# jiwoon-ahn/irn

Measured on AMD Instinct MI355X. Metric: images/sec for CAM+random-walk label gen, VOC12 512^2 (random-walk label generation stage), higher is better.
Workload: dtype f32

## Files before the change

include/irn_hip.h:

```cpp
#ifndef IRN_HIP_H
#define IRN_HIP_H

#include <stddef.h>
#include <stdint.h>

#ifdef __cplusplus
extern "C" {
#endif

#define IRN_OK 0
#define IRN_ERR_ARG 1
#define IRN_ERR_HIP 2
#define IRN_ERR_STATE 3

#define IRN_MAX_RADIUS 16

int irn_version(void);
const char *irn_last_error(void);

int irn_path_count(int radius, int *n_dirs, int *n_cells);
int irn_path_table(int radius, int order, int32_t *dst_dydx, int32_t *path_start, int32_t *cells_dydx);

int irn_edge_to_affinity(const float *edge_dev, int batch, int hp, int wp, int radius,
                         float *aff_dev, void *stream);
// ... 23 lines not shown
                       const int32_t *c, size_t *workspace_bytes);
int irn_walk_run(irn_walk_ctx *ctx, const float *const *edge_dev, const float *const *cam_dev,
                 const int32_t *const *inst_map_dev, const int32_t *k_inst,
                 float *const *out_dev, float beta, int n_sweeps,
                 void *workspace_dev, size_t workspace_bytes, void *stream);

int irn_walk_steps(irn_walk_ctx *ctx, int n_sweeps, int *n_steps);
int irn_power_series(int n, int tol_exp, double *coef_out, int coef_cap, int *n_steps, int *recurrence);

int irn_walk_set_option(irn_walk_ctx *ctx, const char *name, int value);

int irn_walk_sync(irn_walk_ctx *ctx, int *fell_back);
int irn_walk_check(irn_walk_ctx *ctx);
int irn_walk_fallback_runs(irn_walk_ctx *ctx);

int irn_walk_tuning(irn_walk_ctx *ctx, int *poll_delay, int *placement, float *probe_ms4);

int irn_walk_plan_rounds(int radius, int n_images, const int32_t *h, const int32_t *w, const int32_t *channels,
                         int n_workgroups, int placement, int32_t *jobs_out, int cap_rounds, int *n_rounds);

int irn_walk_read_profile(irn_walk_ctx *ctx, long long *host_out);

int irn_walk_enable_timing(irn_walk_ctx *ctx, int enable);
int irn_walk_last_sweep_ms(irn_walk_ctx *ctx, float *ms, int *n_launches);

int irn_walk_export_weights(irn_walk_ctx *ctx, int image, float *w_dev, double *inv_deg_dev,
                            void *workspace_dev, void *stream);

int irn_label_epilogue(int n_images, const float *const *rw_dev, const int32_t *c, const int32_t *h,
                       const int32_t *w, const int32_t *out_h, const int32_t *out_w, float bg_thres,
                       const int64_t *const *keys_dev, uint8_t *const *labels_dev,
                       int32_t *const *argmax_dev, float *const *rw_up_dev, void *scratch_dev,
                       void *stream);

int irn_cam_merge(int n_scales, const float *const *src_dev, const int32_t *hs, const int32_t *ws, int n_classes,
                  const int64_t *keys_dev, int n_keys, int out_h, int out_w, float *cam_dev, float *high_res_dev,
                  void *scratch_dev, void *stream);

int irn_bicubic_plan(int in_size, int out_size, int32_t *ksize, int32_t *lo, int32_t *count, int32_t *weights,
                     size_t weights_capacity);
size_t irn_bicubic_scratch_bytes(int h, int w, int hs, int ws, int channels);
int irn_bicubic_resize_u8(const uint8_t *img_dev, int h, int w, int channels, int hs, int ws, uint8_t *out_dev,
                          void *scratch_dev, void *stream);
int irn_msf_pack(const uint8_t *img_dev, int h, int w, int n_scales, const int32_t *hs, const int32_t *ws,
                 const float *lut_dev, float *const *out_dev, void *scratch_dev, void *stream);

#define IRN_AUGMENT_DESC_WORDS 16
int irn_augment_batch(int n_images, int crop, const int32_t *meta, size_t meta_words, const uint8_t *pixels_dev,
                      size_t pixels_bytes, const float *lut_dev, float *out_dev, size_t out_elems, void *scratch_dev,
                      size_t scratch_bytes, int32_t *meta_dev, size_t meta_dev_words, void *stream);

#define IRN_AUGMENT_LABEL_DESC_WORDS 12
int irn_augment_label_batch(int n_images, int crop, int reduce, const int32_t *meta, size_t meta_words,
                            const uint8_t *labels_dev, size_t labels_bytes, uint8_t *out_dev, size_t out_elems,
                            int32_t *meta_dev, size_t meta_dev_words, void *stream);

int irn_bn_act(float *x_dev, const float *res_dev, const float *scale_dev, const float *shift_dev, const float *res_scale_dev,
               const float *res_shift_dev, int64_t n_images, int n_channels, int64_t plane_elems, int relu, void *stream);

int irn_bn_act_nhwc(float *x_dev, const float *res_dev, const float *scale_dev, const float *shift_dev, const float *res_scale_dev,
                    const float *res_shift_dev, int64_t n_pixels, int n_channels, int relu, void *stream);

int irn_bn_fold(const float *weight_dev, const float *bias_dev, const float *mean_dev, const float *var_dev, double eps,
                int n_channels, float *scale_dev, float *shift_dev, void *stream);
int irn_bn_act_forward(const float *x_dev, const float *res_dev, const float *scale_dev, const float *shift_dev,
                       const float *res_scale_dev, const float *res_shift_dev, float *out_dev, int64_t n_images, int n_channels,
// ... 118 lines not shown
```

irn_amd/_lib.py:

```python
import ctypes as C
import os

import torch

_HERE = os.path.dirname(os.path.abspath(__file__))
LIB_PATH = os.environ.get("IRN_HIP_LIB") or os.path.join(_HERE, "lib", "libirn_hip.so")

if not os.path.exists(LIB_PATH):
    raise ImportError(
        "irn_amd: %s not found — the HIP extension is the product path and has no fallback; "
        "build it with `make -C irn_amd/csrc` (needs hipcc, targets gfx950)" % LIB_PATH)

lib = C.CDLL(LIB_PATH)

vp, i32, f32, sz, i64 = C.c_void_p, C.c_int, C.c_float, C.c_size_t, C.c_int64
pi32 = C.POINTER(C.c_int32)
ppv = C.POINTER(C.c_void_p)

_SIGS = {
    "irn_version": (C.c_int, []),
    "irn_last_error": (C.c_char_p, []),
    "irn_path_count": (i32, [i32, C.POINTER(i32), C.POINTER(i32)]),
    "irn_path_table": (i32, [i32, i32, pi32, pi32, pi32]),
    "irn_edge_to_affinity": (i32, [vp, i32, i32, i32, i32, vp, vp]),
    "irn_edge_to_affinity_backward": (i32, [vp, vp, i32, i32, i32, i32, vp, vp]),
    "irn_pair_displacement": (i32, [vp, i32, i32, i32, i32, i32, vp, vp]),
    "irn_pair_displacement_backward": (i32, [vp, i32, i32, i32, i32, i32, vp, vp]),
    "irn_aff_loss_workspace_bytes": (sz, [i32, i32, i32, i32]),
    "irn_aff_loss_forward": (i32, [vp, vp, vp, i32, i32, i32, i32, vp, vp, vp, sz, vp]),
    "irn_aff_loss_backward": (i32, [vp, vp, vp, i32, i32, i32, i32, vp, vp, vp, vp, sz, vp]),
    "irn_aff_loss_backward_ordered": (i32, [vp, vp, vp, i32, i32, i32, i32, vp, vp, vp, vp, sz, vp]),
    "irn_walk_create": (i32, [i32, C.POINTER(vp)]),
    "irn_walk_destroy": (i32, [vp]),
    "irn_walk_configure": (i32, [vp, i32, pi32, pi32, pi32, C.POINTER(sz)]),
    "irn_walk_run": (i32, [vp, ppv, ppv, ppv, pi32, ppv, f32, i32, vp, sz, vp]),
    "irn_walk_set_option": (i32, [vp, C.c_char_p, i32]),
    "irn_walk_steps": (i32, [vp, i32, C.POINTER(i32)]),
    "irn_power_series": (i32, [i32, i32, C.POINTER(C.c_double), i32, C.POINTER(i32), C.POINTER(i32)]),
    "irn_walk_sync": (i32, [vp, C.POINTER(i32)]),
    "irn_walk_check": (i32, [vp]),
    "irn_walk_fallback_runs": (i32, [vp]),
    "irn_walk_tuning": (i32, [vp, C.POINTER(i32), C.POINTER(i32), C.POINTER(f32)]),
    "irn_walk_plan_rounds": (i32, [i32, i32, pi32, pi32, pi32, i32, i32, pi32, i32, C.POINTER(i32)]),
    "irn_walk_read_profile": (i32, [vp, vp]),
    "irn_walk_enable_timing": (i32, [vp, i32]),
    "irn_walk_last_sweep_ms": (i32, [vp, C.POINTER(f32), C.POINTER(i32)]),
    "irn_walk_export_weights": (i32, [vp, i32, vp, vp, vp, vp]),
    "irn_label_epilogue": (i32, [i32, ppv, pi32, pi32, pi32, pi32, pi32, f32, ppv, ppv, ppv, ppv, vp, vp]),
    "irn_cam_merge": (i32, [i32, ppv, pi32, pi32, i32, vp, i32, i32, i32, vp, vp, vp, vp]),
    "irn_bicubic_plan": (i32, [i32, i32, pi32, pi32, pi32, pi32, sz]),
    "irn_bicubic_scratch_bytes": (sz, [i32, i32, i32, i32, i32]),
    "irn_bicubic_resize_u8": (i32, [vp, i32, i32, i32, i32, i32, vp, vp, vp]),
    "irn_msf_pack": (i32, [vp, i32, i32, i32, pi32, pi32, vp, ppv, vp, vp]),
    "irn_augment_batch": (i32, [i32, i32, pi32, sz, vp, sz, vp, vp, sz, vp, sz, vp, sz, vp]),
    "irn_augment_label_batch": (i32, [i32, i32, i32, pi32, sz, vp, sz, vp, sz, vp, sz, vp]),
    "irn_bn_act": (i32, [vp, vp, vp, vp, vp, vp, i64, i32, i64, i32, vp]),
    "irn_bn_act_nhwc": (i32, [vp, vp, vp, vp, vp, vp, i64, i32, i32, vp]),
    "irn_bn_fold": (i32, [vp, vp, vp, vp, C.c_double, i32, vp, vp, vp]),
    "irn_bn_act_forward": (i32, [vp, vp, vp, vp, vp, vp, vp, i64, i32, i64, i32, vp]),
    "irn_bn_act_backward_workspace_bytes": (sz, [i64, i32, i64]),
    "irn_bn_act_backward": (i32, [vp, vp, vp, vp, vp, vp, vp, vp, vp, i64, i32, i64, i32, vp, sz, vp]),
    "irn_conv1x1_workspace_bytes": (sz, []),
    "irn_conv1x1_algo_count": (i32, [i64, i32, i32, i32, i32, i32, sz, C.POINTER(i32)]),
    "irn_conv1x1_nhwc": (i32, [vp, vp, vp, vp, vp, i64, i32, i32, i32, i32, vp, sz, vp]),
    "irn_split16": (i32, [vp, vp, vp, i32, vp, i64, i32, vp, vp]),
    "irn_split16_pad": (i32, [vp, vp, vp, i32, vp, i64, i32, i32, i32, i32, i32, vp, vp]),
    "irn_conv3x3_split_gemm": (i32, [vp, vp, vp, i64, i32, i32, i32, i32, f32, i32, i32, vp, sz, vp]),
    "irn_gemm16_algo_count": (i32, [i64, i32, i32, i32, i32, i32, sz, C.POINTER(i32)]),
    "irn_gemm16_nhwc": (i32, [vp, vp, vp, vp, vp, i64, i32, i32, i32, f32, i32, vp, sz, vp]),
    "irn_stem_pool": (i32, [vp, vp, vp, i64, i32, i32, i32, vp, vp]),
    "irn_upsample_bilinear": (i32, [vp, i64, i32, i32, i32, i32, vp, vp]),
    "irn_upsample_bilinear_backward": (i32, [vp, vp, i64, i32, i32, i32, i32, vp, vp]),
    "irn_find_centroids": (i32, [vp, i32, i32, i32, vp, vp]),
    "irn_cluster_scratch_bytes": (sz, [i32, i32]),
    "irn_cluster_centroids": (i32, [vp, vp, i32, i32, f32, vp, C.POINTER(i32), vp, vp]),
    "irn_find_centroids_batch": (i32, [i32, ppv, pi32, pi32, i32, ppv, vp]),
    "irn_cluster_batch_scratch_bytes": (sz, [i32, pi32, pi32]),
    "irn_cluster_centroids_batch": (i32, [i32, ppv, ppv, pi32, pi32, f32, ppv, vp, vp, vp]),
    "irn_ccl_scratch_bytes": (sz, [i32, i32, i32]),
    "irn_label4": (i32, [vp, i32, i32, i32, vp, vp, vp, vp]),
    "irn_detect_scratch_bytes": (sz, [i32, i32, i32]),
# ... 70 lines not shown
```

irn_amd/csrc/label.hip:

```cpp
#include "kernels.hpp"

#pragma clang fp contract(off)

namespace irn {

struct LabelJob {
    const float *rw;
    const int64_t *keys;
    uint8_t *labels;
    int32_t *argmax;
    float *rw_up;
    unsigned *max_slot;
    int c, h, w, oh, ow;
    const uint8_t *gt;
};

namespace {

__device__ __forceinline__ unsigned enc_ordered(float f) {
    const unsigned b = __float_as_uint(f);
    return (b & 0x80000000u) ? ~b : (b | 0x80000000u);
}
__device__ __forceinline__ float dec_ordered(unsigned u) {
    return __uint_as_float((u & 0x80000000u) ? (u & 0x7fffffffu) : ~u);
}

struct Taps {
    int i0, i1;
    float l0, l1;
};

__device__ __forceinline__ Taps taps_x4(int dst, int n_in) {
    float src = ((float)dst + 0.5f) * 0.25f;
    src = src - 0.5f;
    src = src < 0.f ? 0.f : src;
    Taps t;
    t.i0 = min((int)src, n_in - 1);
    t.i1 = min(t.i0 + 1, n_in - 1);
    t.l1 = src - (float)t.i0;
    t.l0 = 1.0f - t.l1;
    return t;
}

__device__ __forceinline__ float bilerp(const float *__restrict__ plane, int w, const Taps &ty, const Taps &tx) {
    const float v00 = plane[ty.i0 * w + tx.i0], v01 = plane[ty.i0 * w + tx.i1];
    const float v10 = plane[ty.i1 * w + tx.i0], v11 = plane[ty.i1 * w + tx.i1];
    const float p01 = v01 * tx.l1, p11 = v11 * tx.l1;
    const float top = __builtin_fmaf(v00, tx.l0, p01);
    const float bot = __builtin_fmaf(v10, tx.l0, p11);
    const float pb = ty.l1 * bot;
    return __builtin_fmaf(ty.l0, top, pb);
}

__device__ __forceinline__ int cell_lo(int k) { return k == 0 ? 0 : 4 * k + 2; }

template <int PASS>
__global__ __launch_bounds__(256) void upsample_max_kernel(const LabelJob *__restrict__ jobs) {
    const LabelJob J = jobs[blockIdx.y];
    const unsigned plane_px = (unsigned)(J.h * J.w), cells = (unsigned)J.c * plane_px;
    const float lower = PASS == 2 ? dec_ordered(*J.max_slot) : 0.f;
    float m = -INFINITY;
    for (unsigned i = blockIdx.x * 256 + threadIdx.x; i < cells; i += gridDim.x * 256) {
        const int c = (int)(i / plane_px);
        const int r = (int)(i - (unsigned)c * plane_px);
        const int k = (int)((unsigned)r / (unsigned)J.w), l = r - k * J.w;
        const int y0 = cell_lo(k), x0 = cell_lo(l);
        if (y0 >= J.oh || x0 >= J.ow) continue;
        const float *plane = J.rw + (long)c * J.h * J.w;
        if (PASS == 1) {
            m = fmaxf(m, bilerp(plane, J.w, taps_x4(y0, J.h), taps_x4(x0, J.w)));
        } else {
            const int k1 = min(k + 1, J.h - 1), l1 = min(l + 1, J.w - 1);
            const float u = fmaxf(fmaxf(plane[k * J.w + l], plane[k * J.w + l1]), fmaxf(plane[k1 * J.w + l], plane[k1 * J.w + l1]));
            if (u + fabsf(u) * 1e-6f + 1e-37f < lower) continue;
            const int y1 = min(k == J.h - 1 ? 4 * J.h - 1 : 4 * k + 5, J.oh - 1);
            const int x1 = min(l == J.w - 1 ? 4 * J.w - 1 : 4 * l + 5, J.ow - 1);
            for (int oy = y0; oy <= y1; ++oy) {
                const Taps ty = taps_x4(oy, J.h);
                for (int ox = x0; ox <= x1; ++ox) m = fmaxf(m, bilerp(plane, J.w, ty, taps_x4(ox, J.w)));
            }
        }
    }
    for (int s = 32; s > 0; s >>= 1) m = fmaxf(m, __shfl_xor(m, s));
    __shared__ float wmax[4];
    if ((threadIdx.x & 63) == 0) wmax[threadIdx.x >> 6] = m;
    __syncthreads();
    if (threadIdx.x == 0) {
        m = fmaxf(fmaxf(wmax[0], wmax[1]), fmaxf(wmax[2], wmax[3]));
        if (m > -INFINITY) atomicMax(J.max_slot, enc_ordered(m));
    }
}

__device__ __forceinline__ float bilerp_vals(float v00, float v01, float v10, float v11, const Taps &ty, const Taps &tx) {
    const float p01 = v01 * tx.l1, p11 = v11 * tx.l1;
    const float top = __builtin_fmaf(v00, tx.l0, p01);
    const float bot = __builtin_fmaf(v10, tx.l0, p11);
    const float pb = ty.l1 * bot;
    return __builtin_fmaf(ty.l0, top, pb);
}

__global__ __launch_bounds__(256) void label_argmax_kernel(const LabelJob *__restrict__ jobs, float bg) {
    const LabelJob J = jobs[blockIdx.y];
    const unsigned gw = (unsigned)(J.ow + 3) >> 2, groups = gw * (unsigned)J.oh;
    const unsigned npx = (unsigned)J.oh * (unsigned)J.ow;
    const float gmax = dec_ordered(*J.max_slot);
    for (unsigned g = blockIdx.x * 256 + threadIdx.x; g < groups; g += gridDim.x * 256) {
        const int oy = (int)(g / gw), ox = (int)(g - (unsigned)oy * gw) * 4;
        const int nq = min(4, J.ow - ox);
        const Taps ty = taps_x4(oy, J.h);
        Taps tx[4];
#pragma unroll
        for (int q = 0; q < 4; ++q) tx[q] = taps_x4(min(ox + q, J.ow - 1), J.w);
        float best[4] = {bg, bg, bg, bg};
        int idx[4] = {0, 0, 0, 0};
        const unsigned o = (unsigned)oy * (unsigned)J.ow + (unsigned)ox;
        for (int c = 0; c < J.c; ++c) {
            const float *r0 = J.rw + (long)c * J.h * J.w + ty.i0 * J.w, *r1 = J.rw + (long)c * J.h * J.w + ty.i1 * J.w;
            const float a00 = r0[tx[0].i0], a01 = r0[tx[0].i1], a10 = r1[tx[0].i0], a11 = r1[tx[0].i1];
// ... 5 lines not shown
            v[3] = bilerp_vals(b00, b01, b10, b11, ty, tx[3]) / gmax;
            if (J.rw_up) {
                float *dst = J.rw_up + (long)c * npx + o;
                if (nq == 4 && ((uintptr_t)dst & 15) == 0) *reinterpret_cast<float4 *>(dst) = make_float4(v[0], v[1], v[2], v[3]);
                else
                    for (int q = 0; q < nq; ++q) dst[q] = v[q];
            }
#pragma unroll
            for (int q = 0; q < 4; ++q)
                if (v[q] > best[q] || (v[q] != v[q] && best[q] == best[q])) {
                    best[q] = v[q];
                    idx[q] = c + 1;
                }
        }
        if (J.argmax) {
            int32_t *dst = J.argmax + o;
            if (nq == 4 && ((uintptr_t)dst & 15) == 0) *reinterpret_cast<int4 *>(dst) = make_int4(idx[0], idx[1], idx[2], idx[3]);
            else
                for (int q = 0; q < nq; ++q) dst[q] = idx[q];
        }
        if (J.labels) {
            uint8_t lab[4];
#pragma unroll
            for (int q = 0; q < 4; ++q) lab[q] = idx[q] == 0 ? (uint8_t)0 : (uint8_t)(J.keys[idx[q] - 1] + 1);
            uint8_t *dst = J.labels + o;
            if (nq == 4 && ((uintptr_t)dst & 3) == 0)
                *reinterpret_cast<uint32_t *>(dst) = (uint32_t)lab[0] | ((uint32_t)lab[1] << 8) | ((uint32_t)lab[2] << 16) | ((uint32_t)lab[3] << 24);
            else
                for (int q = 0; q < nq; ++q) dst[q] = lab[q];
        }
    }
}

constexpr int kSweepGroups = 4;
constexpr int kSweepChunk = 256 * kSweepGroups;
constexpr int kSweepCap = 15360;
constexpr int kSweepRows = IRN_EVAL_CLASSES + 1;
constexpr int kSweepMaxC = IRN_EVAL_CLASSES - 1;
constexpr uint32_t kSweepSkip = 0xffffffffu;

__global__ __launch_bounds__(256) void label_sweep_kernel(const LabelJob *__restrict__ jobs, const float *__restrict__ thres,
                                                          int t, int cap, int64_t *__restrict__ hist, int64_t *__restrict__ bad) {
    extern __shared__ __attribute__((aligned(16))) uint32_t sweep_lds[];
    uint32_t *bins = sweep_lds;
    float *th = reinterpret_cast<float *>(sweep_lds + cap);
    int *col = reinterpret_cast<int *>(th + IRN_EVAL_MAX_THRES);
    uint32_t *nbad = reinterpret_cast<uint32_t *>(col + kSweepMaxC);
    const LabelJob J = jobs[blockIdx.y];
    const int tid = threadIdx.x;
    if (tid == 0) *nbad = 0;
    for (int i = tid; i < t; i += 256) th[i] = thres[i];
    if (tid < J.c) {
        const int64_t key = J.keys[tid];
        col[tid] = (key >= 0 && key < kSweepMaxC) ? (int)key + 1 : -1;
    }
    __syncthreads();
    uint32_t local_bad = 0;
    if (blockIdx.x == 0 && blockIdx.y == 0)
        for (int i = tid; i < t; i += 256)
            if (th[i] != th[i] || (i > 0 && !(th[i - 1] <= th[i]))) ++local_bad;

    const unsigned gw = (unsigned)(J.ow + 3) >> 2, groups = gw * (unsigned)J.oh;
    const unsigned chunks = (groups + kSweepChunk - 1) / kSweepChunk;
    const uint32_t nbins = (uint32_t)(t + 1) * kSweepRows * (uint32_t)J.c;
    const float gmax = dec_ordered(*J.max_slot);
    for (unsigned chunk = blockIdx.x; chunk < chunks; chunk += gridDim.x) {
// ... 122 lines not shown
        const int oy = (int)(o / ow), ox = (int)(o - (long)oy * ow);
        float acc = 0.f;
        for (int s = 0; s < A.n_scales; ++s) {
            const Taps ty = taps_resize(oy, A.hs[s], th), tx = taps_resize(ox, A.ws[s], tw);
            acc = acc + bilerp(A.src[s] + (long)cls * A.hs[s] * A.ws[s], A.ws[s], ty, tx);
        }
        out[o] = acc;
        m = fmaxf(m, acc);
    }
    for (int s = 32; s > 0; s >>= 1) m = fmaxf(m, __shfl_xor(m, s));
    __shared__ float wmax[4];
    if ((threadIdx.x & 63) == 0) wmax[threadIdx.x >> 6] = m;
    __syncthreads();
    if (threadIdx.x == 0) {
        m = fmaxf(fmaxf(wmax[0], wmax[1]), fmaxf(wmax[2], wmax[3]));
        if (m > -INFINITY) atomicMax(A.max_slots + (is_hi ? A.k : 0) + kk, enc_ordered(m));
    }
}

__global__ __launch_bounds__(256) void cam_merge_norm_kernel(const MergeArgs A) {
    const int kk = blockIdx.y;
    const bool is_hi = blockIdx.z == 1;
    const long n = is_hi ? (long)A.H * A.W : (long)A.lh * A.lw;
    float *out = (is_hi ? A.hi : A.lo) + (long)kk * n;
    const float den = dec_ordered(A.max_slots[(is_hi ? A.k : 0) + kk]) + 1e-5f;
    for (long o = (long)blockIdx.x * 256 + threadIdx.x; o < n; o += (long)gridDim.x * 256) out[o] = out[o] / den;
}

}
}

using namespace irn;

extern "C" int irn_label_epilogue(int n_images, const float *const *rw_dev, const int32_t *c, const int32_t *h,
                                  const int32_t *w, const int32_t *out_h, const int32_t *out_w, float bg_thres,
                                  const int64_t *const *keys_dev, uint8_t *const *labels_dev,
                                  int32_t *const *argmax_dev, float *const *rw_up_dev, void *scratch_dev,
                                  void *stream_) {
    hipStream_t stream = (hipStream_t)stream_;
    if (n_images < 1 || !rw_dev || !c || !h || !w || !out_h || !out_w || !scratch_dev)
        return fail(IRN_ERR_ARG, "irn_label_epilogue: bad argument");
    std::vector<LabelJob> jobs(n_images);
    long max_px = 0, max_cells = 0;
    for (int i = 0; i < n_images; ++i) {
        LabelJob &J = jobs[i];
        if (!rw_dev[i] || c[i] < 1 || h[i] < 1 || w[i] < 1 || out_h[i] < 1 || out_w[i] < 1 ||
            out_h[i] > 4 * h[i] || out_w[i] > 4 * w[i])
            return fail(IRN_ERR_ARG, "irn_label_epilogue: image %d: bad sizes (c=%d %dx%d -> %dx%d)", i, c[i], h[i],
                        w[i], out_h[i], out_w[i]);
        J.rw = rw_dev[i];
        J.keys = keys_dev ? keys_dev[i] : nullptr;
        J.labels = labels_dev ? labels_dev[i] : nullptr;
        J.argmax = argmax_dev ? argmax_dev[i] : nullptr;
        J.rw_up = rw_up_dev ? rw_up_dev[i] : nullptr;
        if (J.labels && !J.keys)
            return fail(IRN_ERR_ARG, "irn_label_epilogue: image %d: labels requested without keys", i);
        J.max_slot = (unsigned *)scratch_dev + i;
        J.c = c[i]; J.h = h[i]; J.w = w[i]; J.oh = out_h[i]; J.ow = out_w[i];
        max_px = std::max(max_px, (long)out_h[i] * out_w[i]);
        max_cells = std::max(max_cells, (long)c[i] * h[i] * w[i]);
    }
    LabelJob *jobs_dev = nullptr;
    int rc = scratch_upload(jobs.data(), sizeof(LabelJob) * n_images, (void **)&jobs_dev, stream);
    if (rc) return rc;
    IRN_HIP_TRY(hipMemsetAsync(scratch_dev, 0, sizeof(unsigned) * n_images, stream));
    if (max_px >= (1L << 31) || max_cells >= (1L << 31)) return fail(IRN_ERR_ARG, "irn_label_epilogue: image too large (32-bit pixel indices)");
    const long per_image = std::max<long>(1, 4096 / n_images);
    const int bx = (int)std::min<long>((max_px / 4 + 255) / 256 + 1, 512);
    const int bc = (int)std::min<long>((max_cells + 255) / 256, per_image);
    hipLaunchKernelGGL(upsample_max_kernel<1>, dim3(bc, n_images), dim3(256), 0, stream, jobs_dev);
    IRN_LAUNCH_CHECK("upsample_max_kernel<1>");
    hipLaunchKernelGGL(upsample_max_kernel<2>, dim3(bc, n_images), dim3(256), 0, stream, jobs_dev);
    IRN_LAUNCH_CHECK("upsample_max_kernel<2>");
    hipLaunchKernelGGL(label_argmax_kernel, dim3(bx, n_images), dim3(256), 0, stream, jobs_dev, bg_thres);
    IRN_LAUNCH_CHECK("label_argmax_kernel");
    return scratch_release(stream);
}

extern "C" int irn_label_sweep_confusion(int n_images, const float *const *rw_dev, const int32_t *c, const int32_t *h,
                                         const int32_t *w, const int32_t *out_h, const int32_t *out_w,
                                         const int64_t *const *keys_dev, const uint8_t *const *gt_dev,
                                         const float *thres_dev, int t, int64_t *hist_dev, int64_t *bad_dev,
                                         void *scratch_dev, void *stream_) {
    hipStream_t stream = (hipStream_t)stream_;
    if (n_images < 1 || n_images > 65535 || !rw_dev || !c || !h || !w || !out_h || !out_w || !keys_dev || !gt_dev || !thres_dev ||
        !hist_dev || !bad_dev || !scratch_dev || t < 1 || t > IRN_EVAL_MAX_THRES)
        return fail(IRN_ERR_ARG, "irn_label_sweep_confusion: bad argument (n_images=%d, t=%d; 1 <= t <= %d)", n_images, t,
                    IRN_EVAL_MAX_THRES);
    std::vector<LabelJob> jobs(n_images);
    long max_px = 0, max_cells = 0;
    int max_c = 0;
    for (int i = 0; i < n_images; ++i) {
        LabelJob &J = jobs[i];
        if (!rw_dev[i] || c[i] < 1 || c[i] > kSweepMaxC || h[i] < 1 || w[i] < 1 || out_h[i] < 1 || out_w[i] < 1 ||
            out_h[i] > 4 * h[i] || out_w[i] > 4 * w[i])
            return fail(IRN_ERR_ARG, "irn_label_sweep_confusion: image %d: bad sizes (c=%d %dx%d -> %dx%d; 1 <= c <= %d)", i,
                        c[i], h[i], w[i], out_h[i], out_w[i], kSweepMaxC);
        if (!keys_dev[i] || !gt_dev[i])
            return fail(IRN_ERR_ARG, "irn_label_sweep_confusion: image %d: keys and ground truth are required", i);
        J.rw = rw_dev[i];
        J.keys = keys_dev[i];
        J.labels = nullptr;
        J.argmax = nullptr;
        J.rw_up = nullptr;
        J.gt = gt_dev[i];
        J.max_slot = (unsigned *)scratch_dev + i;
        J.c = c[i]; J.h = h[i]; J.w = w[i]; J.oh = out_h[i]; J.ow = out_w[i];
        max_px = std::max(max_px, (long)out_h[i] * out_w[i]);
        max_cells = std::max(max_cells, (long)c[i] * h[i] * w[i]);
        max_c = std::max(max_c, c[i]);
    }
    if (max_px >= (1L << 31) || max_cells >= (1L << 31))
        return fail(IRN_ERR_ARG, "irn_label_sweep_confusion: image too large (32-bit pixel indices)");
    LabelJob *jobs_dev = nullptr;
    int rc = scratch_upload(jobs.data(), sizeof(LabelJob) * n_images, (void **)&jobs_dev, stream);
    if (rc) return rc;
    IRN_HIP_TRY(hipMemsetAsync(scratch_dev, 0, sizeof(unsigned) * n_images, stream));
    const long per_image = std::max<long>(1, 4096 / n_images);
    const int bc = (int)std::min<long>((max_cells + 255) / 256, per_image);
    hipLaunchKernelGGL(upsample_max_kernel<1>, dim3(bc, n_images), dim3(256), 0, stream, jobs_dev);
    IRN_LAUNCH_CHECK("upsample_max_kernel<1>");
    hipLaunchKernelGGL(upsample_max_kernel<2>, dim3(bc, n_images), dim3(256), 0, stream, jobs_dev);
    IRN_LAUNCH_CHECK("upsample_max_kernel<2>");
    const long nbins = (long)(t + 1) * kSweepRows * max_c;
    const int cap = (int)std::min<long>((nbins + 3) / 4 * 4, kSweepCap);
    const size_t lds = sizeof(uint32_t) * cap + sizeof(float) * IRN_EVAL_MAX_THRES + sizeof(int) * kSweepMaxC + sizeof(uint32_t);
    const int bx = (int)std::min<long>(((max_px + 3) / 4 + kSweepChunk - 1) / kSweepChunk + 1, 128);
    hipLaunchKernelGGL(label_sweep_kernel, dim3(bx, n_images), dim3(256), lds, stream, jobs_dev, thres_dev, t, cap, hist_dev,
                       bad_dev);
    IRN_LAUNCH_CHECK("label_sweep_kernel");
    return scratch_release(stream);
}

extern "C" int irn_cam_merge(int n_scales, const float *const *src_dev, const int32_t *hs, const int32_t *ws, int n_classes,
                             const int64_t *keys_dev, int n_keys, int out_h, int out_w, float *cam_dev,
                             float *high_res_dev, void *scratch_dev, void *stream_) {
    hipStream_t stream = (hipStream_t)stream_;
    if (n_scales < 1 || n_scales > kMaxScales || !src_dev || !hs || !ws || n_classes < 1 || !keys_dev || n_keys < 1 ||
        out_h < 1 || out_w < 1 || !cam_dev || !high_res_dev || !scratch_dev)
        return fail(IRN_ERR_ARG, "irn_cam_merge: bad argument (1..%d scales, >= 1 key)", kMaxScales);
    MergeArgs A;
    for (int s = 0; s < n_scales; ++s) {
        if (!src_dev[s] || hs[s] < 1 || ws[s] < 1) return fail(IRN_ERR_ARG, "irn_cam_merge: scale %d: bad input", s);
        A.src[s] = src_dev[s];
        A.hs[s] = hs[s];
        A.ws[s] = ws[s];
    }
    A.n_scales = n_scales;
    A.n_cls = n_classes;
    A.k = n_keys;
    A.keys = keys_dev;
    A.lo = cam_dev;
    A.hi = high_res_dev;
    A.H = out_h;
    A.W = out_w;
    A.lh = (out_h - 1) / 4 + 1;
// ... 13 lines not shown
```

irn_amd/ops.py:

```python
import collections
import ctypes as C

import numpy as np
import torch

from ._lib import _need_cuda, _need_vec, _stream, check, i32_array, lib, ptr_array
from .gemm import (conv1x1_algo_count, conv1x1_nhwc, conv3x3_split, gemm16_algo_count, gemm16_nhwc, gemm_ranks, gemm_ranks16,
                   gemm_ranks3x3, split16, split16_pad, split_overflowed, split_weight, split_weight_3x3)


def label_epilogue(rws, out_sizes, bg_thres, keys=None, want_labels=True, want_argmax=False, want_rw_up=False, packed=False):
    n = len(rws)
    dev = rws[0].device
    rs, cs, hs, ws, ohs, ows = [], [], [], [], [], []
    for i in range(n):
        _need_cuda(rws[i], "rw")
        r = rws[i].reshape((-1,) + tuple(rws[i].shape[-2:])).contiguous().float()
        rs.append(r)
        cs.append(r.shape[0]); hs.append(r.shape[1]); ws.append(r.shape[2])
        ohs.append(int(out_sizes[i][0])); ows.append(int(out_sizes[i][1]))
    labels = flat = None
    if want_labels and packed:
        offs = np.concatenate([[0], np.cumsum([ohs[i] * ows[i] for i in range(n)])])
        flat = torch.empty(int(offs[-1]), dtype=torch.uint8, device=dev)
        labels = [flat[int(offs[i]):int(offs[i + 1])].view(ohs[i], ows[i]) for i in range(n)]
    elif want_labels:
        labels = [torch.empty((ohs[i], ows[i]), dtype=torch.uint8, device=dev) for i in range(n)]
    argmax = [torch.empty((ohs[i], ows[i]), dtype=torch.int32, device=dev) for i in range(n)] if want_argmax else None
    rw_up = [torch.empty((cs[i], ohs[i], ows[i]), dtype=torch.float32, device=dev) for i in range(n)] if want_rw_up else None
    ks = None
    if want_labels:
        if keys is None:
            raise ValueError("labels need keys")
        ks = [torch.as_tensor(k, device=dev).to(torch.int64).contiguous() for k in keys]
    scratch = torch.empty(max(n, 64), dtype=torch.int32, device=dev)
    with torch.cuda.device(dev):
        check(lib.irn_label_epilogue(
            n, ptr_array([r.data_ptr() for r in rs]), i32_array(cs), i32_array(hs), i32_array(ws),
            i32_array(ohs), i32_array(ows), float(bg_thres),
            None if ks is None else ptr_array([k.data_ptr() for k in ks]),
            None if labels is None else ptr_array([t.data_ptr() for t in labels]),
            None if argmax is None else ptr_array([t.data_ptr() for t in argmax]),
            None if rw_up is None else ptr_array([t.data_ptr() for t in rw_up]),
            scratch.data_ptr(), _stream()))
    out = {}
    if want_labels:
        out["labels"] = labels
        if flat is not None:
            out["labels_flat"] = flat
    if want_argmax:
        out["argmax"] = argmax
    if want_rw_up:
        out["rw_up"] = rw_up
    return out


def cam_merge(outputs, size, label):
    for o in outputs:
        _need_cuda(o, "CAM output")
    dev = outputs[0].device
    outs = [o.contiguous().float() for o in outputs]
    n_cls = outs[0].shape[0]
    H, W = int(size[0]), int(size[1])
    label = torch.as_tensor(label)
    if label.is_cuda:
        keys = torch.nonzero(label.to(dev))[:, 0].to(torch.int64).contiguous()
    else:
        keys = torch.nonzero(label)[:, 0].to(torch.int64).contiguous().to(dev, non_blocking=True)
    k = int(keys.numel())
    cam = torch.empty((k, (H - 1) // 4 + 1, (W - 1) // 4 + 1), dtype=torch.float32, device=dev)
    hi = torch.empty((k, H, W), dtype=torch.float32, device=dev)
    scratch = torch.empty(2 * k, dtype=torch.int32, device=dev)
    with torch.cuda.device(dev):
        check(lib.irn_cam_merge(len(outs), ptr_array([o.data_ptr() for o in outs]), i32_array([o.shape[1] for o in outs]),
                                i32_array([o.shape[2] for o in outs]), n_cls, keys.data_ptr(), k, H, W, cam.data_ptr(),
                                hi.data_ptr(), scratch.data_ptr(), _stream()))
    return keys, cam, hi

# ... 1167 lines not shown
```

Measured before the change: 19560.

## Single-pass row-wise upsample max and tiled fast label argmax kernel

Replaces the two-pass upsample-max (a coarse pass plus a pruned exact pass) with one wave-per-row pass. It precomputes the vertical taps and computes each cell's exact upsampled maximum directly. When no rw_up output is requested, it also replaces the per-pixel label argmax kernel with a tiled kernel. That kernel handles 4x4 output blocks per thread, reuses separable bilinear partial sums across channels, and prefetches the next channel's taps. The background test uses a precomputed threshold instead of dividing by the max. Near-ties, NaNs and unsafe thresholds fall back to the exact per-pixel path, and an optional slow-path counter is added. This adds code complexity and relies on the threshold and tie-margin logic matching the reference exactly.

```diff
diff --git a/include/irn_hip.h b/include/irn_hip.h
--- a/include/irn_hip.h
+++ b/include/irn_hip.h
@@ -79,6 +79,11 @@
                        const int64_t *const *keys_dev, uint8_t *const *labels_dev,
                        int32_t *const *argmax_dev, float *const *rw_up_dev, void *scratch_dev,
                        void *stream);
+int irn_label_epilogue_counted(int n_images, const float *const *rw_dev, const int32_t *c, const int32_t *h,
+                               const int32_t *w, const int32_t *out_h, const int32_t *out_w, float bg_thres,
+                               const int64_t *const *keys_dev, uint8_t *const *labels_dev,
+                               int32_t *const *argmax_dev, float *const *rw_up_dev, void *scratch_dev,
+                               uint32_t *slow_count_dev, void *stream);
 
 int irn_cam_merge(int n_scales, const float *const *src_dev, const int32_t *hs, const int32_t *ws, int n_classes,
                   const int64_t *keys_dev, int n_keys, int out_h, int out_w, float *cam_dev, float *high_res_dev,
diff --git a/irn_amd/_lib.py b/irn_amd/_lib.py
--- a/irn_amd/_lib.py
+++ b/irn_amd/_lib.py
@@ -47,6 +47,7 @@
     "irn_walk_last_sweep_ms": (i32, [vp, C.POINTER(f32), C.POINTER(i32)]),
     "irn_walk_export_weights": (i32, [vp, i32, vp, vp, vp, vp]),
     "irn_label_epilogue": (i32, [i32, ppv, pi32, pi32, pi32, pi32, pi32, f32, ppv, ppv, ppv, ppv, vp, vp]),
+    "irn_label_epilogue_counted": (i32, [i32, ppv, pi32, pi32, pi32, pi32, pi32, f32, ppv, ppv, ppv, ppv, vp, vp, vp]),
     "irn_cam_merge": (i32, [i32, ppv, pi32, pi32, i32, vp, i32, i32, i32, vp, vp, vp, vp]),
     "irn_bicubic_plan": (i32, [i32, i32, pi32, pi32, pi32, pi32, sz]),
     "irn_bicubic_scratch_bytes": (sz, [i32, i32, i32, i32, i32]),
diff --git a/irn_amd/csrc/label.hip b/irn_amd/csrc/label.hip
--- a/irn_amd/csrc/label.hip
+++ b/irn_amd/csrc/label.hip
@@ -13,6 +13,7 @@
     unsigned *max_slot;
     int c, h, w, oh, ow;
     const uint8_t *gt;
+    unsigned *slow_count;
 };
 
 namespace {
@@ -24,6 +25,8 @@
 __device__ __forceinline__ float dec_ordered(unsigned u) {
     return __uint_as_float((u & 0x80000000u) ? (u & 0x7fffffffu) : ~u);
 }
+
+typedef __attribute__((address_space(1))) const float global_cfloat;
 
 struct Taps {
     int i0, i1;
@@ -53,37 +56,65 @@
 }
 
 __device__ __forceinline__ int cell_lo(int k) { return k == 0 ? 0 : 4 * k + 2; }
-
-template <int PASS>
+__device__ __forceinline__ int cell_hi(int k, int n_in, int n_out) { return min(k == n_in - 1 ? 4 * n_in - 1 : 4 * k + 5, n_out - 1); }
+
+__device__ __forceinline__ float cell_max(float m, float v00, float v01, float v10, float v11, int x0, int x1, int w,
+                                          const float (&ly0)[6], const float (&ly1)[6], int n_rows) {
+    for (int ox = x0; ox <= x1; ++ox) {
+        const Taps tx = taps_x4(ox, w);
+        const float p01 = v01 * tx.l1, p11 = v11 * tx.l1;
+        const float top = __builtin_fmaf(v00, tx.l0, p01);
+        const float bot = __builtin_fmaf(v10, tx.l0, p11);
+#pragma unroll
+        for (int r = 0; r < 6; ++r)
+            if (r < n_rows) {
+                const float pb = ly1[r] * bot;
+                m = fmaxf(m, __builtin_fmaf(ly0[r], top, pb));
+            }
+    }
+    return m;
+}
+
 __global__ __launch_bounds__(256) void upsample_max_kernel(const LabelJob *__restrict__ jobs) {
     const LabelJob J = jobs[blockIdx.y];
-    const unsigned plane_px = (unsigned)(J.h * J.w), cells = (unsigned)J.c * plane_px;
-    const float lower = PASS == 2 ? dec_ordered(*J.max_slot) : 0.f;
+    const int lane = threadIdx.x & 63;
+    const int n_waves = (int)gridDim.x * 4;
+    int k = __builtin_amdgcn_readfirstlane((int)blockIdx.x * 4 + (int)(threadIdx.x >> 6)), c = 0;
     float m = -INFINITY;
-    for (unsigned i = blockIdx.x * 256 + threadIdx.x; i < cells; i += gridDim.x * 256) {
-        const int c = (int)(i / plane_px);
-        const int r = (int)(i - (unsigned)c * plane_px);
-        const int k = (int)((unsigned)r / (unsigned)J.w), l = r - k * J.w;
-        const int y0 = cell_lo(k), x0 = cell_lo(l);
-        if (y0 >= J.oh || x0 >= J.ow) continue;
-        const float *plane = J.rw + (long)c * J.h * J.w;
-        if (PASS == 1) {
-            m = fmaxf(m, bilerp(plane, J.w, taps_x4(y0, J.h), taps_x4(x0, J.w)));
-        } else {
-            const int k1 = min(k + 1, J.h - 1), l1 = min(l + 1, J.w - 1);
-            const float u = fmaxf(fmaxf(plane[k * J.w + l], plane[k * J.w + l1]), fmaxf(plane[k1 * J.w + l], plane[k1 * J.w + l1]));
-            if (u + fabsf(u) * 1e-6f + 1e-37f < lower) continue;
-            const int y1 = min(k == J.h - 1 ? 4 * J.h - 1 : 4 * k + 5, J.oh - 1);
-            const int x1 = min(l == J.w - 1 ? 4 * J.w - 1 : 4 * l + 5, J.ow - 1);
-            for (int oy = y0; oy <= y1; ++oy) {
-                const Taps ty = taps_x4(oy, J.h);
-                for (int ox = x0; ox <= x1; ++ox) m = fmaxf(m, bilerp(plane, J.w, ty, taps_x4(ox, J.w)));
-            }
-        }
+    for (;;) {
+        while (k >= J.h && c < J.c) {
+            k -= J.h;
+            ++c;
+        }
+        if (c >= J.c) break;
+        const int y0 = cell_lo(k);
+        if (y0 < J.oh) {
+            const int n_rows = cell_hi(k, J.h, J.oh) - y0 + 1;
+            float ly0[6], ly1[6];
+#pragma unroll
+            for (int r = 0; r < 6; ++r) {
+                const Taps ty = taps_x4(min(y0 + r, J.oh - 1), J.h);
+                ly0[r] = ty.l0;
+                ly1[r] = ty.l1;
+            }
+            global_cfloat *r0 = (global_cfloat *)(J.rw + ((long)c * J.h + k) * J.w);
+            global_cfloat *r1 = (global_cfloat *)(J.rw + ((long)c * J.h + min(k + 1, J.h - 1)) * J.w);
+            for (int l = lane; l < J.w; l += 128) {
+                const int x0 = cell_lo(l);
+                if (x0 >= J.ow) break;
+                const int lb = l + 64, lb_c = min(lb, J.w - 1);
+                const int l1 = min(l + 1, J.w - 1), lb1 = min(lb_c + 1, J.w - 1);
+                const float a00 = r0[l], a01 = r0[l1], a10 = r1[l], a11 = r1[l1];
+                const float b00 = r0[lb_c], b01 = r0[lb1], b10 = r1[lb_c], b11 = r1[lb1];
+                m = cell_max(m, a00, a01, a10, a11, x0, cell_hi(l, J.w, J.ow), J.w, ly0, ly1, n_rows);
+                if (lb < J.w && cell_lo(lb) < J.ow) m = cell_max(m, b00, b01, b10, b11, cell_lo(lb), cell_hi(lb, J.w, J.ow), J.w, ly0, ly1, n_rows);
+            }
+        }
+        k += n_waves;
     }
     for (int s = 32; s > 0; s >>= 1) m = fmaxf(m, __shfl_xor(m, s));
     __shared__ float wmax[4];
-    if ((threadIdx.x & 63) == 0) wmax[threadIdx.x >> 6] = m;
+    if (lane == 0) wmax[threadIdx.x >> 6] = m;
     __syncthreads();
     if (threadIdx.x == 0) {
         m = fmaxf(fmaxf(wmax[0], wmax[1]), fmaxf(wmax[2], wmax[3]));
@@ -155,6 +186,235 @@
     }
 }
 
+struct FastImage {
+    float T;
+    bool ok;
+};
+
+__device__ __forceinline__ FastImage fast_threshold(float gmax, float bg) {
+    const bool pre = gmax >= 0x1p-100f && gmax < INFINITY && bg >= 0x1p-20f && bg < 1.0f;
+    const unsigned lane = threadIdx.x & 63u;
+    const unsigned bits = __float_as_uint(bg * gmax) + lane - 32u;
+    const float cand = __uint_as_float(bits);
+    const unsigned long long above = __ballot(cand / gmax > bg);
+    const int first = above ? __ffsll((long long)above) - 1 : 0;
+    FastImage F;
+    F.ok = pre && first > 0 && above == (~0ull << first);
+    F.T = __uint_as_float(__float_as_uint(bg * gmax) + (unsigned)first - 32u);
+    return F;
+}
+
+constexpr float kTieMargin = 1.0f - 0x1p-19f;
+
+__device__ __forceinline__ int decide_pixel(const LabelJob &J, int oy, int ox, float bg, float gmax, const FastImage &F, unsigned &slow) {
+    const Taps ty = taps_x4(oy, J.h), tx = taps_x4(ox, J.w);
+    const long plane = (long)J.h * J.w;
+    if (F.ok) {
+        float m = -INFINITY, runner = -INFINITY;
+        int c1 = 0;
+        bool nan = false;
+        for (int c = 0; c < J.c; ++c) {
+            const float v = bilerp(J.rw + c * plane, J.w, ty, tx);
+            nan = nan || v != v;
+            if (v > m) {
+                runner = m;
+                m = v;
+                c1 = c;
+            }
+        }
+        if (!nan) {
+            if (m < F.T) return 0;
+            if (!(runner >= m * kTieMargin)) return c1 + 1;
+        }
+    }
+    ++slow;
+    float best = bg;
+    int idx = 0;
+    for (int c = 0; c < J.c; ++c) {
+        const float v = bilerp(J.rw + c * plane, J.w, ty, tx) / gmax;
+        if (v > best || (v != v && best == best)) {
+            best = v;
+            idx = c + 1;
+        }
+    }
+    return idx;
+}
+
+struct FastTile {
+    int i, j;
+    bool valid;
+    int s0, s1, s2, c0, c1, c2;
+    bool y_mid, x_mid;
+    float ly0[4], ly1[4], lx0[4], lx1[4];
+};
+
+__device__ __forceinline__ FastTile fast_tile(const LabelJob &J, int tile_y, int tile_x, int gh, int gw) {
+    FastTile A;
+    A.i = tile_y * 4 + (int)(threadIdx.x >> 6);
+    A.j = tile_x * 64 + (int)(threadIdx.x & 63);
+    A.valid = A.i < gh && A.j < gw;
+    const int i = min(A.i, gh - 1), j = min(A.j, gw - 1);
+    Taps ty[4], tx[4];
+#pragma unroll
+    for (int q = 0; q < 4; ++q) {
+        ty[q] = taps_x4(4 * i + q, J.h);
+        tx[q] = taps_x4(4 * j + q, J.w);
+        A.ly0[q] = ty[q].l0; A.ly1[q] = ty[q].l1;
+        A.lx0[q] = tx[q].l0; A.lx1[q] = tx[q].l1;
+    }
+    A.s0 = ty[0].i0 * J.w; A.s1 = ty[0].i1 * J.w; A.s2 = ty[2].i1 * J.w;
+    A.c0 = tx[0].i0; A.c1 = tx[0].i1; A.c2 = tx[2].i1;
+    A.y_mid = ty[2].i0 == ty[0].i1;
+    A.x_mid = tx[2].i0 == tx[0].i1;
+    return A;
+}
+
+__device__ __forceinline__ void fast_load(float (&a)[9], const float *__restrict__ p_, const FastTile &A) {
+    global_cfloat *p = (global_cfloat *)p_;
+    a[0] = p[A.s0 + A.c0]; a[1] = p[A.s0 + A.c1]; a[2] = p[A.s0 + A.c2];
+    a[3] = p[A.s1 + A.c0]; a[4] = p[A.s1 + A.c1]; a[5] = p[A.s1 + A.c2];
+    a[6] = p[A.s2 + A.c0]; a[7] = p[A.s2 + A.c1]; a[8] = p[A.s2 + A.c2];
+}
+
+constexpr int kKeyTab = 256;
+
+__global__ __launch_bounds__(256) __attribute__((amdgpu_waves_per_eu(4))) void label_fast_kernel(const LabelJob *__restrict__ jobs, float bg) {
+    __shared__ uint8_t keytab[kKeyTab + 1];
+    const LabelJob J = jobs[blockIdx.y];
+    const int gw = (J.ow + 3) >> 2, gh = (J.oh + 3) >> 2;
+    const int tiles_x = (gw + 63) >> 6, tiles_y = (gh + 3) >> 2;
+    const long plane = (long)J.h * J.w;
+    unsigned slow = 0;
+    int tx_ = (int)blockIdx.x, ty_ = 0;
+    while (tx_ >= tiles_x && ty_ < tiles_y) {
+        tx_ -= tiles_x;
+        ++ty_;
+    }
+    bool more = ty_ < tiles_y;
+    FastTile A = fast_tile(J, more ? ty_ : 0, more ? tx_ : 0, gh, gw);
+    float a[9];
+    fast_load(a, J.rw, A);
+    __builtin_amdgcn_sched_barrier(0);
+    const unsigned gmax_bits = *(const __attribute__((address_space(1))) unsigned *)J.max_slot;
+    if (J.labels) {
+        const int t = (int)threadIdx.x + 1;
+        if (threadIdx.x == 0) keytab[0] = 0;
+        if (t <= min(J.c, kKeyTab)) keytab[t] = (uint8_t)(J.keys[t - 1] + 1);
+    }
+    __syncthreads();
+    const float gmax = dec_ordered(gmax_bits);
+    const FastImage F = fast_threshold(gmax, bg);
+    while (more) {
+        const int oy = 4 * A.i, ox = 4 * A.j;
+        const int nr = A.valid ? min(4, J.oh - oy) : 0, nq = min(4, J.ow - ox);
+        float m[16], det = 0.f;
+        unsigned sel[16];
+        bool near[16];
+#pragma unroll
+        for (int n = 0; n < 16; ++n) {
+            m[n] = -INFINITY;
+            sel[n] = 0;
+            near[n] = false;
+        }
+        for (int c = 0; c < J.c; ++c) {
+            const unsigned sc = (unsigned)(c + 1);
+            float b[9];
+            fast_load(b, J.rw + min(c + 1, J.c - 1) * plane, A);
+            float H[3][4];
+#pragma unroll
+            for (int s = 0; s < 3; ++s) {
+#pragma unroll
+                for (int t = 0; t < 3; ++t) det = __builtin_fmaf(a[3 * s + t], 0.f, det);
+                const float left = A.x_mid ? a[3 * s + 1] : a[3 * s];
+#pragma unroll
+                for (int q = 0; q < 4; ++q) {
+                    const float v0 = q < 2 ? a[3 * s] : left, v1 = q < 2 ? a[3 * s + 1] : a[3 * s + 2];
+                    const float p1 = v1 * A.lx1[q];
+                    H[s][q] = __builtin_fmaf(v0, A.lx0[q], p1);
+                }
+            }
+#pragma unroll
+            for (int r = 0; r < 4; ++r)
+#pragma unroll
+                for (int q = 0; q < 4; ++q) {
+                    const float top = r < 2 ? H[0][q] : (A.y_mid ? H[1][q] : H[0][q]), bot = r < 2 ? H[1][q] : H[2][q];
+                    const float pb = A.ly1[r] * bot;
+                    const float v = __builtin_fmaf(A.ly0[r], top, pb);
+                    const int n = 4 * r + q;
+                    const bool up = v > m[n];
+                    near[n] = up ? m[n] >= v * kTieMargin : near[n];
+                    m[n] = up ? v : m[n];
+                    sel[n] = up ? sc : sel[n];
+                }
+#pragma unroll
+            for (int t = 0; t < 9; ++t) a[t] = b[t];
+        }
+        unsigned res[16], again = 0;
+#pragma unroll
+        for (int n = 0; n < 16; ++n) {
+            const bool is_bg = m[n] < F.T;
+            res[n] = is_bg ? 0u : sel[n];
+            if (!is_bg && near[n]) again |= 1u << n;
+        }
+        if (!F.ok || det != det) again = 0xffffu;
+        const unsigned o = (unsigned)oy * (unsigned)J.ow + (unsigned)ox;
+#pragma unroll
+        for (int r = 0; r < 4; ++r) {
+            if (r >= nr) continue;
+            const unsigned orow = o + (unsigned)r * (unsigned)J.ow;
+            if (J.argmax) {
+                int32_t *dst = J.argmax + orow;
+                if (nq == 4 && ((uintptr_t)dst & 15) == 0)
+                    *reinterpret_cast<int4 *>(dst) = make_int4((int)res[4 * r], (int)res[4 * r + 1], (int)res[4 * r + 2], (int)res[4 * r + 3]);
+                else {
+#pragma unroll
+                    for (int q = 0; q < 4; ++q)
+                        if (q < nq) dst[q] = (int)res[4 * r + q];
+                }
+            }
+            if (J.labels) {
+                uint8_t lab[4];
+#pragma unroll
+                for (int q = 0; q < 4; ++q) {
+                    const unsigned e = res[4 * r + q];
+                    lab[q] = e <= (unsigned)kKeyTab ? keytab[e] : (uint8_t)(J.keys[e - 1] + 1);
+                }
+                uint8_t *dst = J.labels + orow;
+                if (nq == 4 && ((uintptr_t)dst & 3) == 0)
+                    *(__attribute__((address_space(1))) uint32_t *)dst = (uint32_t)lab[0] | ((uint32_t)lab[1] << 8) | ((uint32_t)lab[2] << 16) | ((uint32_t)lab[3] << 24);
+                else {
+#pragma unroll
+                    for (int q = 0; q < 4; ++q)
+                        if (q < nq) dst[q] = lab[q];
+                }
+            }
+        }
+        if (again)
+            for (int n = 0; n < 16; ++n) {
+                const int r = n >> 2, q = n & 3;
+                if (!((again >> n) & 1u) || r >= nr || q >= nq) continue;
+                const int idx = decide_pixel(J, oy + r, ox + q, bg, gmax, F, slow);
+                const unsigned on = o + (unsigned)r * (unsigned)J.ow + (unsigned)q;
+                if (J.argmax) J.argmax[on] = idx;
+                if (J.labels) J.labels[on] = idx == 0 ? (uint8_t)0 : (uint8_t)(J.keys[idx - 1] + 1);
+            }
+        tx_ += (int)gridDim.x;
+        while (tx_ >= tiles_x && ty_ < tiles_y) {
+            tx_ -= tiles_x;
+            ++ty_;
+        }
+        more = ty_ < tiles_y;
+        if (more) {
+            A = fast_tile(J, ty_, tx_, gh, gw);
+            fast_load(a, J.rw, A);
+        }
+    }
+    if (J.slow_count) {
+        for (int s = 32; s > 0; s >>= 1) slow += __shfl_xor(slow, s);
+        if ((threadIdx.x & 63) == 0 && slow) atomicAdd(J.slow_count, slow);
+    }
+}
+
 constexpr int kSweepGroups = 4;
 constexpr int kSweepChunk = 256 * kSweepGroups;
 constexpr int kSweepCap = 15360;
@@ -343,16 +603,25 @@
 
 using namespace irn;
 
-extern "C" int irn_label_epilogue(int n_images, const float *const *rw_dev, const int32_t *c, const int32_t *h,
-                                  const int32_t *w, const int32_t *out_h, const int32_t *out_w, float bg_thres,
-                                  const int64_t *const *keys_dev, uint8_t *const *labels_dev,
-                                  int32_t *const *argmax_dev, float *const *rw_up_dev, void *scratch_dev,
-                                  void *stream_) {
+static int launch_upsample_max(const LabelJob *jobs_dev, int n_images, long max_rows, hipStream_t stream) {
+    const long per_image = std::max<long>(1, 4096 / n_images);
+    const int bc = (int)std::min<long>((max_rows + 3) / 4, per_image);
+    hipLaunchKernelGGL(upsample_max_kernel, dim3(bc, n_images), dim3(256), 0, stream, jobs_dev);
+    IRN_LAUNCH_CHECK("upsample_max_kernel");
+    return IRN_OK;
+}
+
+static int label_epilogue_impl(int n_images, const float *const *rw_dev, const int32_t *c, const int32_t *h,
+                               const int32_t *w, const int32_t *out_h, const int32_t *out_w, float bg_thres,
+                               const int64_t *const *keys_dev, uint8_t *const *labels_dev,
+                               int32_t *const *argmax_dev, float *const *rw_up_dev, void *scratch_dev,
+                               uint32_t *slow_count_dev, void *stream_) {
     hipStream_t stream = (hipStream_t)stream_;
     if (n_images < 1 || !rw_dev || !c || !h || !w || !out_h || !out_w || !scratch_dev)
         return fail(IRN_ERR_ARG, "irn_label_epilogue: bad argument");
     std::vector<LabelJob> jobs(n_images);
-    long max_px = 0, max_cells = 0;
+    long max_px = 0, max_cells = 0, max_rows = 0, max_tiles = 0;
+    bool any_rw_up = false;
     for (int i = 0; i < n_images; ++i) {
         LabelJob &J = jobs[i];
         if (!rw_dev[i] || c[i] < 1 || h[i] < 1 || w[i] < 1 || out_h[i] < 1 || out_w[i] < 1 ||
@@ -367,25 +636,51 @@
         if (J.labels && !J.keys)
             return fail(IRN_ERR_ARG, "irn_label_epilogue: image %d: labels requested without keys", i);
         J.max_slot = (unsigned *)scratch_dev + i;
+        J.slow_count = slow_count_dev ? slow_count_dev + i : nullptr;
         J.c = c[i]; J.h = h[i]; J.w = w[i]; J.oh = out_h[i]; J.ow = out_w[i];
+        any_rw_up = any_rw_up || J.rw_up;
         max_px = std::max(max_px, (long)out_h[i] * out_w[i]);
         max_cells = std::max(max_cells, (long)c[i] * h[i] * w[i]);
-    }
+        max_rows = std::max(max_rows, (long)c[i] * h[i]);
+        max_tiles = std::max(max_tiles, (((long)out_w[i] + 3) / 4 + 63) / 64 * ((((long)out_h[i] + 3) / 4 + 3) / 4));
+    }
+    if (max_px >= (1L << 31) || max_cells >= (1L << 31)) return fail(IRN_ERR_ARG, "irn_label_epilogue: image too large (32-bit pixel indices)");
     LabelJob *jobs_dev = nullptr;
     int rc = scratch_upload(jobs.data(), sizeof(LabelJob) * n_images, (void **)&jobs_dev, stream);
     if (rc) return rc;
     IRN_HIP_TRY(hipMemsetAsync(scratch_dev, 0, sizeof(unsigned) * n_images, stream));
-    if (max_px >= (1L << 31) || max_cells >= (1L << 31)) return fail(IRN_ERR_ARG, "irn_label_epilogue: image too large (32-bit pixel indices)");
-    const long per_image = std::max<long>(1, 4096 / n_images);
-    const int bx = (int)std::min<long>((max_px / 4 + 255) / 256 + 1, 512);
-    const int bc = (int)std::min<long>((max_cells + 255) / 256, per_image);
-    hipLaunchKernelGGL(upsample_max_kernel<1>, dim3(bc, n_images), dim3(256), 0, stream, jobs_dev);
-    IRN_LAUNCH_CHECK("upsample_max_kernel<1>");
-    hipLaunchKernelGGL(upsample_max_kernel<2>, dim3(bc, n_images), dim3(256), 0, stream, jobs_dev);
-    IRN_LAUNCH_CHECK("upsample_max_kernel<2>");
-    hipLaunchKernelGGL(label_argmax_kernel, dim3(bx, n_images), dim3(256), 0, stream, jobs_dev, bg_thres);
-    IRN_LAUNCH_CHECK("label_argmax_kernel");
+    if (slow_count_dev) IRN_HIP_TRY(hipMemsetAsync(slow_count_dev, 0, sizeof(uint32_t) * n_images, stream));
+    rc = launch_upsample_max(jobs_dev, n_images, max_rows, stream);
+    if (rc) return rc;
+    if (any_rw_up) {
+        const int bx = (int)std::min<long>((max_px / 4 + 255) / 256 + 1, 512);
+        hipLaunchKernelGGL(label_argmax_kernel, dim3(bx, n_images), dim3(256), 0, stream, jobs_dev, bg_thres);
+        IRN_LAUNCH_CHECK("label_argmax_kernel");
+    } else {
+        const int bx = (int)std::min<long>(max_tiles, 128);
+        hipLaunchKernelGGL(label_fast_kernel, dim3(bx, n_images), dim3(256), 0, stream, jobs_dev, bg_thres);
+        IRN_LAUNCH_CHECK("label_fast_kernel");
+    }
     return scratch_release(stream);
+}
+
+extern "C" int irn_label_epilogue(int n_images, const float *const *rw_dev, const int32_t *c, const int32_t *h,
+                                  const int32_t *w, const int32_t *out_h, const int32_t *out_w, float bg_thres,
+                                  const int64_t *const *keys_dev, uint8_t *const *labels_dev,
+                                  int32_t *const *argmax_dev, float *const *rw_up_dev, void *scratch_dev,
+                                  void *stream) {
+    return label_epilogue_impl(n_images, rw_dev, c, h, w, out_h, out_w, bg_thres, keys_dev, labels_dev, argmax_dev, rw_up_dev,
+                               scratch_dev, nullptr, stream);
+}
+
+extern "C" int irn_label_epilogue_counted(int n_images, const float *const *rw_dev, const int32_t *c, const int32_t *h,
+                                          const int32_t *w, const int32_t *out_h, const int32_t *out_w, float bg_thres,
+                                          const int64_t *const *keys_dev, uint8_t *const *labels_dev,
+                                          int32_t *const *argmax_dev, float *const *rw_up_dev, void *scratch_dev,
+                                          uint32_t *slow_count_dev, void *stream) {
+    if (!slow_count_dev) return fail(IRN_ERR_ARG, "irn_label_epilogue_counted: no counter array");
+    return label_epilogue_impl(n_images, rw_dev, c, h, w, out_h, out_w, bg_thres, keys_dev, labels_dev, argmax_dev, rw_up_dev,
+                               scratch_dev, slow_count_dev, stream);
 }
 
 extern "C" int irn_label_sweep_confusion(int n_images, const float *const *rw_dev, const int32_t *c, const int32_t *h,
@@ -399,7 +694,7 @@
         return fail(IRN_ERR_ARG, "irn_label_sweep_confusion: bad argument (n_images=%d, t=%d; 1 <= t <= %d)", n_images, t,
                     IRN_EVAL_MAX_THRES);
     std::vector<LabelJob> jobs(n_images);
-    long max_px = 0, max_cells = 0;
+    long max_px = 0, max_cells = 0, max_rows = 0;
     int max_c = 0;
     for (int i = 0; i < n_images; ++i) {
         LabelJob &J = jobs[i];
@@ -419,6 +714,7 @@
         J.c = c[i]; J.h = h[i]; J.w = w[i]; J.oh = out_h[i]; J.ow = out_w[i];
         max_px = std::max(max_px, (long)out_h[i] * out_w[i]);
         max_cells = std::max(max_cells, (long)c[i] * h[i] * w[i]);
+        max_rows = std::max(max_rows, (long)c[i] * h[i]);
         max_c = std::max(max_c, c[i]);
     }
     if (max_px >= (1L << 31) || max_cells >= (1L << 31))
@@ -427,12 +723,8 @@
     int rc = scratch_upload(jobs.data(), sizeof(LabelJob) * n_images, (void **)&jobs_dev, stream);
     if (rc) return rc;
     IRN_HIP_TRY(hipMemsetAsync(scratch_dev, 0, sizeof(unsigned) * n_images, stream));
-    const long per_image = std::max<long>(1, 4096 / n_images);
-    const int bc = (int)std::min<long>((max_cells + 255) / 256, per_image);
-    hipLaunchKernelGGL(upsample_max_kernel<1>, dim3(bc, n_images), dim3(256), 0, stream, jobs_dev);
-    IRN_LAUNCH_CHECK("upsample_max_kernel<1>");
-    hipLaunchKernelGGL(upsample_max_kernel<2>, dim3(bc, n_images), dim3(256), 0, stream, jobs_dev);
-    IRN_LAUNCH_CHECK("upsample_max_kernel<2>");
+    rc = launch_upsample_max(jobs_dev, n_images, max_rows, stream);
+    if (rc) return rc;
     const long nbins = (long)(t + 1) * kSweepRows * max_c;
     const int cap = (int)std::min<long>((nbins + 3) / 4 * 4, kSweepCap);
     const size_t lds = sizeof(uint32_t) * cap + sizeof(float) * IRN_EVAL_MAX_THRES + sizeof(int) * kSweepMaxC + sizeof(uint32_t);
diff --git a/irn_amd/ops.py b/irn_amd/ops.py
--- a/irn_amd/ops.py
+++ b/irn_amd/ops.py
@@ -9,7 +9,8 @@
                    gemm_ranks3x3, split16, split16_pad, split_overflowed, split_weight, split_weight_3x3)
 
 
-def label_epilogue(rws, out_sizes, bg_thres, keys=None, want_labels=True, want_argmax=False, want_rw_up=False, packed=False):
+def label_epilogue(rws, out_sizes, bg_thres, keys=None, want_labels=True, want_argmax=False, want_rw_up=False, packed=False,
+                   count_slow=False):
     n = len(rws)
     dev = rws[0].device
     rs, cs, hs, ws, ohs, ows = [], [], [], [], [], []
@@ -34,16 +35,22 @@
             raise ValueError("labels need keys")
         ks = [torch.as_tensor(k, device=dev).to(torch.int64).contiguous() for k in keys]
     scratch = torch.empty(max(n, 64), dtype=torch.int32, device=dev)
-    with torch.cuda.device(dev):
-        check(lib.irn_label_epilogue(
-            n, ptr_array([r.data_ptr() for r in rs]), i32_array(cs), i32_array(hs), i32_array(ws),
-            i32_array(ohs), i32_array(ows), float(bg_thres),
-            None if ks is None else ptr_array([k.data_ptr() for k in ks]),
-            None if labels is None else ptr_array([t.data_ptr() for t in labels]),
-            None if argmax is None else ptr_array([t.data_ptr() for t in argmax]),
-            None if rw_up is None else ptr_array([t.data_ptr() for t in rw_up]),
-            scratch.data_ptr(), _stream()))
+    slow = torch.empty(n, dtype=torch.int32, device=dev) if count_slow else None
+    with torch.cuda.device(dev):
+        args = (n, ptr_array([r.data_ptr() for r in rs]), i32_array(cs), i32_array(hs), i32_array(ws),
+                i32_array(ohs), i32_array(ows), float(bg_thres),
+                None if ks is None else ptr_array([k.data_ptr() for k in ks]),
+                None if labels is None else ptr_array([t.data_ptr() for t in labels]),
+                None if argmax is None else ptr_array([t.data_ptr() for t in argmax]),
+                None if rw_up is None else ptr_array([t.data_ptr() for t in rw_up]),
+                scratch.data_ptr())
+        if count_slow:
+            check(lib.irn_label_epilogue_counted(*args, slow.data_ptr(), _stream()))
+        else:
+            check(lib.irn_label_epilogue(*args, _stream()))
     out = {}
+    if count_slow:
+        out["slow_count"] = slow
     if want_labels:
         out["labels"] = labels
         if flat is not None:
```

After: 19640 (median of 6 runs). Within noise of the previous version (+0.4%).
